# CaptainEven/DenseBox

Hardware: AMD Instinct MI355X
Metric: training patches/sec (240x240) (higher is better)
Workload: dtype f16; 1 GPU; full training step (fwd + fused dense loss w/ hard-negative mining + bwd + grad all-reduce + SGD) of DenseBoxLMLOC on 240x240 patches; net=DenseBoxLMLOC, batch_per_gpu=64, global_batch=64, patch=240x240, parallelism=dp1, half_neg=11, grad_finite=True

## Files before the change

densebox_amd/_lib.py:

```python
import ctypes as C
import os

_HERE = os.path.dirname(os.path.abspath(__file__))
LIB_PATH = os.environ.get('DBX_LIB') or os.path.join(_HERE, 'csrc', 'libdensebox_hip.so')

F16, BF16, F32 = 0, 1, 2
DTYPE_ID = {'f16': F16, 'bf16': BF16, 'f32': F32}
ESIZE = {F16: 2, BF16: 2, F32: 4}

EPI_BIAS, EPI_RELU, EPI_GATE, EPI_DROPMASK, EPI_ACCUM, EPI_F32_NCHW, EPI_DROPHASH = 1, 2, 4, 8, 16, 32, 64
CONV_WFRAG = 128
K_IGEMM, K_DMA, K_BAND, K_C64, K_C8, K_WS, K_P8 = 1, 2, 3, 4, 5, 6, 7


class View(C.Structure):
    _fields_ = [('ptr', C.c_void_p), ('n', C.c_int32), ('h', C.c_int32), ('w', C.c_int32),
                ('pad', C.c_int32), ('ld', C.c_int32), ('c_off', C.c_int32), ('c', C.c_int32)]


class ConvDesc(C.Structure):
    _fields_ = [('dtype', C.c_int32), ('kh', C.c_int32), ('kw', C.c_int32), ('cpad', C.c_int32),
                ('cin_pad', C.c_int32), ('cout_pad', C.c_int32), ('epilogue', C.c_int32), ('drop_seed', C.c_uint32)]


# ... 178 lines not shown
    'dbx_dp_allreduce_sum_f32': (C.c_int, [_VP, _VP, _I64, _VP]),
    'dbx_dp_destroy': (C.c_int, [_VP]),
    'dbx_conv_dgrad_wgrad1_scratch_bytes': (_I64, []),
    'dbx_conv_dgrad_wgrad1_fusable': (C.c_int, [_PC, _PV, _PV, _PV]),
    'dbx_conv_dgrad_wgrad1': (C.c_int, [_PC, _PV, _VP, _PV, _PV, _I32, _VP, _VP, _VP, _I32, _VP]),
    'dbx_conv_pool_fusable': (C.c_int, [_PC, _PV, _PV]),
    'dbx_conv_forward_pool': (C.c_int, [_PC, _PV, _VP, _VP, _PV, _PV, _I32, _VP]),
    'dbx_conv_forward_pool_idx': (C.c_int, [_PC, _PV, _VP, _VP, _PV, _PV, _I32, _VP, _VP]),
    'dbx_pack_weight': (C.c_int, [_I32, _I32, _VP, _I32, _I32, _I32, _I32, _VP, _I32, _I32, _I32, _I32, _VP]),
    'dbx_fold_heads': (C.c_int, [_VP, _VP, _VP, _VP, _I32, _VP, _VP, _VP]),
    'dbx_fold_refine': (C.c_int, [_VP, _VP, _VP, _VP, _VP, _VP, _I32, _I32, _VP, _VP, _VP, _VP]),
    'dbx_refine_eval': (C.c_int, [_VP, _VP, _I32, _I32, _I32, _VP, _VP, _VP, _VP]),
    'dbx_refine_backward_scratch_bytes': (C.c_int64, [_I32, _I32, _I32]),
    'dbx_refine_backward': (C.c_int, [_VP, _VP, _VP, _I32, _I32, _I32, _VP, _VP, _VP, _VP, _VP, _VP, _I32, _VP, _VP, _VP, _VP, _VP, _VP, _VP, _VP, _VP, _VP, _VP, _VP, _VP, _VP]),
    'dbx_upsample_bilinear_nchw_f32': (C.c_int, [_VP, _I32, _I32, _I32, _VP, _I32, _I32, _VP]),
    'dbx_pack_multi': (C.c_int, [_I32, _VP, _I32, _I64, _VP]),
    'dbx_sgd_pack_step': (C.c_int, [_I32, _VP, _I32, _I64, _VP, _F, _F, _F, _I32, _VP]),
    'dbx_head2_dgrad': (C.c_int, [_I32, _PV, C.POINTER(C.c_void_p), C.POINTER(C.c_int32), _I32, _PV, _VP, _I32, _I32, C.c_uint32, _VP]),
    'dbx_head2_wgrad_scratch_bytes': (_I64, [_I32, _I32]),
    'dbx_head2_wgrad': (C.c_int, [_I32, _PV, _PV, C.POINTER(C.c_int32), _I32, C.POINTER(C.c_void_p), C.POINTER(C.c_void_p), _VP, _VP]),
    'dbx_head2_backward': (C.c_int, [_I32, _PV, _PV, C.POINTER(C.c_void_p), C.POINTER(C.c_int32), _I32, _PV, _VP, _I32, _I32, C.c_uint32,
                                     C.POINTER(C.c_void_p), C.POINTER(C.c_void_p), _VP, _VP]),
    'dbx_head2_backward_up': (C.c_int, [_I32, _PV, _PV, C.POINTER(C.c_void_p), C.POINTER(C.c_int32), _I32, _PV, _VP, _I32, _I32, C.c_uint32,
                                        C.POINTER(C.c_void_p), C.POINTER(C.c_void_p), _VP, _PV, _VP]),
    'dbx_perspective_matrix': (C.c_int, [_VP, _VP, _VP]),
    'dbx_warp_perspective_u8': (C.c_int, [_VP, _I32, _I32, _I32, _VP, _VP, _I32, _I32, _VP]),
    'dbx_warp_batch_workspace_bytes': (_I64, [_I32]),
    'dbx_warp_perspective_batch_u8': (C.c_int, [C.POINTER(WarpJob), _I32, _I32, _VP, _VP, _VP]),
    'dbx_plate_crops_batch': (C.c_int, [_VP, _I32, _I32, _VP, _I64, _I64, _VP, _I32, _I32, _I32, _VP, _VP, _VP, _VP]),
    'dbx_match_gt_batch': (C.c_int, [_VP, _I32, _I64, _VP, _VP, _I32, _I32, _VP, _I32, _VP, _VP, _I32, _D, _VP, _VP, _VP, _VP, _VP, _VP]),
# ... 131 lines not shown
```

densebox_amd/csrc/aux_ops.hip:

```cpp
#include "common.hpp"
#include <mutex>

static thread_local char g_err[512] = "";
void dbx_set_error(const char* fmt, ...) {
    va_list ap;
    va_start(ap, fmt);
    vsnprintf(g_err, sizeof(g_err), fmt, ap);
    va_end(ap);
}
extern "C" const char* dbx_last_error(void) { return g_err; }
extern "C" int dbx_version(void) { return DBX_ABI_VERSION; }
extern "C" int dbx_device_arch(int device) {
    hipDeviceProp_t p;
    if (hipGetDeviceProperties(&p, device) != hipSuccess) { dbx_set_error("hipGetDeviceProperties failed"); return DBX_ERR_HIP; }
    int arch = 0;
    const char* s = p.gcnArchName;
    if (s[0] == 'g' && s[1] == 'f' && s[2] == 'x') arch = (int)strtol(s + 3, nullptr, 16) == 0x950 ? 950 : (int)strtol(s + 3, nullptr, 10);
    return arch;
}

template <typename T> struct Vec { static constexpr int N = 16 / sizeof(T); };

template <typename T> __device__ __forceinline__ void load_vec(const T* p, float (&v)[16 / sizeof(T)]) {
    const u32x4 raw = *(const u32x4*)p;
// ... 1809 lines not shown
            const float bot = lx0 * p[y1 * wi + x0] + lx1 * p[y1 * wi + x1];
            y[i] = ly0 * top + ly1 * bot;
        }
    }
}
extern "C" int dbx_upsample_bilinear_nchw_f32(const float* x, int32_t planes, int32_t hi, int32_t wi, float* y, int32_t ho, int32_t wo,
                                              void* stream) {
    DBX_REQUIRE(x && y && planes >= 1 && hi >= 1 && wi >= 1 && ho >= 1 && wo >= 1, "upsample_nchw: bad arguments");
    const int64_t total = (int64_t)planes * ho * wo;
    hipLaunchKernelGGL(upsample_nchw_f32_kernel, dim3(grid_for(total)), dim3(256), 0, (hipStream_t)stream, x, planes, hi, wi, y, ho, wo,
                       ac_scale(hi, ho), ac_scale(wi, wo));
    DBX_LAUNCH_CHECK();
    return DBX_OK;
}

template <typename T>
__global__ void u8hwc_to_framed_kernel(const unsigned char* __restrict__ x, FrameGeo y, float m0, float m1, float m2, float s0,
                                       float s1, float s2) {
    constexpr int V = Vec<T>::N;
    const int cg = y.c / V;
    const int64_t total = (int64_t)y.n * y.h * y.w;
    for (int64_t i = blockIdx.x * (int64_t)blockDim.x + threadIdx.x; i < total; i += (int64_t)gridDim.x * blockDim.x) {
        const int px = (int)(i % y.w);
        const int py = (int)((i / y.w) % y.h);
        const int n = (int)(i / ((int64_t)y.w * y.h));
        const unsigned char* p = x + i * 3;
        float v[3];
        v[0] = ((float)p[0] / 255.0f - m0) / s0;
        v[1] = ((float)p[1] / 255.0f - m1) / s1;
        v[2] = ((float)p[2] / 255.0f - m2) / s2;
// ... 23 lines not shown
```

densebox_amd/csrc/refine_ops.hip:

```cpp
#include "common.hpp"

namespace {
constexpr int RCI = 5, RTAPS = 49, RG1 = RCI * RTAPS + 1;

__device__ __forceinline__ void rf_coef(int d, float scale, int in, int& i0, int& i1, float& l0, float& l1) {
#pragma clang fp contract(off)
    const float src = scale * (float)d;
    i0 = (int)src;
    if (i0 > in - 1) i0 = in - 1;
    i1 = i0 + (i0 < in - 1 ? 1 : 0);
    l1 = src - (float)i0;
    l0 = 1.f - l1;
}
inline float rf_scale(int in, int out) { return out > 1 ? (float)(in - 1) / (float)(out - 1) : 0.f; }

__global__ void refine_up_t_kernel(const float* __restrict__ d, int n, int ho, int wo, float* __restrict__ g, int hs, int ws, float sy, float sx) {
    const int64_t total = (int64_t)n * hs * ws;
    for (int64_t i = blockIdx.x * (int64_t)blockDim.x + threadIdx.x; i < total; i += (int64_t)gridDim.x * blockDim.x) {
        const int px = (int)(i % ws), py = (int)((i / ws) % hs);
        const int64_t im = i / ((int64_t)ws * hs);
        int ylo = sy > 0.f ? (int)((float)(py - 1) / sy) - 1 : 0, yhi = sy > 0.f ? (int)((float)(py + 1) / sy) + 2 : ho - 1;
        int xlo = sx > 0.f ? (int)((float)(px - 1) / sx) - 1 : 0, xhi = sx > 0.f ? (int)((float)(px + 1) / sx) + 2 : wo - 1;
        ylo = ylo < 0 ? 0 : ylo; xlo = xlo < 0 ? 0 : xlo; yhi = yhi > ho - 1 ? ho - 1 : yhi; xhi = xhi > wo - 1 ? wo - 1 : xhi;
        const float* dp = d + im * ho * wo;
        float acc = 0.f;
        for (int y = ylo; y <= yhi; ++y) {
            int y0, y1; float ly0, ly1;
            rf_coef(y, sy, hs, y0, y1, ly0, ly1);
            const float wy = (y0 == py ? ly0 : 0.f) + (y1 == py ? ly1 : 0.f);
            if (wy == 0.f) continue;
            for (int x = xlo; x <= xhi; ++x) {
                int x0, x1; float lx0, lx1;
                rf_coef(x, sx, ws, x0, x1, lx0, lx1);
                const float wx = (x0 == px ? lx0 : 0.f) + (x1 == px ? lx1 : 0.f);
                if (wx != 0.f) acc = fmaf(wy * wx, dp[y * wo + x], acc);
            }
        }
        g[i] = acc;
    }
}

constexpr int RSPLIT = 4;
__global__ __launch_bounds__(256) void refine_g1_kernel(const float* __restrict__ lm, const float* __restrict__ sc, int h, int w,
                                                        const float* __restrict__ g, float* __restrict__ partial) {
    extern __shared__ float sm[];
    const int ph = h / 2, pw = w / 2, oh = ph - 6, ow = pw - 6;
    const int n = blockIdx.x / RSPLIT, part = blockIdx.x % RSPLIT, tid = threadIdx.x;
    const int rows = (oh + RSPLIT - 1) / RSPLIT, y0 = part * rows < oh ? part * rows : oh, y1 = y0 + rows < oh ? y0 + rows : oh;
    const int xr = y1 > y0 ? y1 - y0 + 6 : 0;
    float* x5 = sm;
    float* gs = sm + RCI * (rows + 6) * pw;
    for (int e = tid; e < RCI * xr * pw; e += 256) {
        const int c = e / (xr * pw), r = e % (xr * pw), py = y0 + r / pw, px = r % pw;
// ... 4 lines not shown
    __syncthreads();
    if (tid < RG1) {
        float acc = 0.f;
        if (tid < RCI * RTAPS) {
            const int c = tid / RTAPS, u = (tid % RTAPS) / 7, v = tid % 7;
            const float* xc = x5 + (c * xr + u) * pw + v;
            for (int y = 0; y < y1 - y0; ++y)
                for (int x = 0; x < ow; ++x) acc = fmaf(gs[y * ow + x], xc[y * pw + x], acc);
        } else {
            for (int e = 0; e < (y1 - y0) * ow; ++e) acc += gs[e];
        }
        partial[(size_t)blockIdx.x * RG1 + tid] = acc;
    }
}

struct RefineW { const float *w1, *b1, *w2, *b2, *w3, *b3, *V; float *dw1, *db1, *dw2, *db2, *dw3, *db3; };
__global__ __launch_bounds__(256) void refine_wgrad_kernel(const float* __restrict__ partial, int nimg, int cm, RefineW a) {
    __shared__ float G1[RG1], G2[64 * 25], V[64 * 25], w1s[64 * RCI * 9], red[256];
    const int tid = threadIdx.x;
    for (int e = tid; e < cm * RCI * 9; e += 256) w1s[e] = a.w1[e];
    if (tid < RG1) {
        float acc = 0.f;
#pragma unroll 16
        for (int n = 0; n < nimg; ++n) acc += partial[(size_t)n * RG1 + tid];
        G1[tid] = acc;
    }
    const int blk = blockIdx.x;
    if (blk == cm)
        for (int e = tid; e < cm * 25; e += 256) V[e] = a.V[e];
    __syncthreads();
    const float Sg = G1[RG1 - 1];
    for (int e = tid; e < cm * 25; e += 256) {
        const int m = e / 25, aa = (e % 25) / 5, bb = e % 5;
        float acc = a.b1[m] * Sg;
        for (int c = 0; c < RCI; ++c)
            for (int i = 0; i < 3; ++i)
                for (int j = 0; j < 3; ++j) acc = fmaf(w1s[(m * RCI + c) * 9 + i * 3 + j], G1[(c * 7 + aa + i) * 7 + bb + j], acc);
        G2[e] = acc;
    }
    __syncthreads();
    if (blk < cm) {
        const int n = blk;
// ... 14 lines not shown
    } else {
        for (int e = tid; e < cm * RCI * 9; e += 256) {
            const int m = e / (RCI * 9), c = (e / 9) % RCI, i = (e % 9) / 3, j = e % 3;
            float acc = 0.f;
            for (int aa = 0; aa < 5; ++aa)
                for (int bb = 0; bb < 5; ++bb) acc = fmaf(V[m * 25 + aa * 5 + bb], G1[(c * 7 + aa + i) * 7 + bb + j], acc);
            a.dw1[e] = acc;
        }
        for (int m = tid; m < cm; m += 256) {
            float sv = 0.f;
            for (int ab = 0; ab < 25; ++ab) sv += V[m * 25 + ab];
            a.db1[m] = sv * Sg;
        }
        if (tid == 0) a.db3[0] = Sg;
    }
}

__global__ void refine_dgrad_kernel(const float* __restrict__ lm, const float* __restrict__ sc, int n, int h, int w, const float* __restrict__ g,
                                    const float* __restrict__ wf, const float* __restrict__ g_lm, const float* __restrict__ g_sc,
                                    float* __restrict__ out_lm, float* __restrict__ out_sc) {
    __shared__ float wsm[RCI * RTAPS];
    for (int e = threadIdx.x; e < RCI * RTAPS; e += blockDim.x) wsm[e] = wf[e];
    __syncthreads();
    const int ph = h / 2, pw = w / 2, oh = ph - 6, ow = pw - 6, wh = (h + 1) / 2, ww = (w + 1) / 2;
    const int64_t total = (int64_t)n * RCI * wh * ww;
    for (int64_t i = blockIdx.x * (int64_t)blockDim.x + threadIdx.x; i < total; i += (int64_t)gridDim.x * blockDim.x) {
        const int wx = (int)(i % ww), wy = (int)((i / ww) % wh), c = (int)((i / ((int64_t)ww * wh)) % RCI);
        const int im = (int)(i / ((int64_t)ww * wh * RCI));
        const size_t plane = c < 4 ? ((size_t)im * 4 + c) * h * w : (size_t)im * h * w;
        const float* xin = (c < 4 ? lm : sc) + plane;
// ... 14 lines not shown
            const float* p = xin + (size_t)(2 * wy) * w + 2 * wx;
            float m = p[0]; arg = 0;
            if (p[1] > m) { m = p[1]; arg = 1; }
            if (p[w] > m) { m = p[w]; arg = 2; }
            if (p[w + 1] > m) { m = p[w + 1]; arg = 3; }
        }
#pragma unroll
        for (int k = 0; k < 4; ++k) {
            const int y = 2 * wy + (k >> 1), x = 2 * wx + (k & 1);
            if (y >= h || x >= w) continue;
            const float in = gin ? gin[(size_t)y * w + x] : 0.f;
            dst[(size_t)y * w + x] = in + (k == arg ? dv : 0.f);
        }
    }
}
}

extern "C" int64_t dbx_refine_backward_scratch_bytes(int32_t n, int32_t h, int32_t w) {
    const int64_t oh = h / 2 - 6, ow = w / 2 - 6;
    return ((int64_t)n * oh * ow + (int64_t)n * RSPLIT * RG1 + 64) * 4;
}

extern "C" int dbx_refine_backward(const float* d_refine, const float* landmark, const float* score, int32_t n, int32_t h, int32_t w,
                                   const float* w1, const float* b1, const float* w2, const float* b2, const float* w3, const float* b3,
                                   int32_t cm, const float* w_fold, const float* v_fold, const float* g_landmark, const float* g_score, float* out_landmark,
                                   float* out_score, float* dw1, float* db1, float* dw2, float* db2, float* dw3, float* db3, void* scratch,
                                   void* stream) {
    DBX_REQUIRE(d_refine && landmark && score && w1 && b1 && w2 && b2 && w3 && b3 && w_fold && v_fold && out_landmark && out_score && dw1 && db1 && dw2 &&
                    db2 && dw3 && db3 && scratch, "refine_backward: null argument");
    DBX_REQUIRE(n >= 1 && h / 2 >= 7 && w / 2 >= 7 && cm >= 1 && cm <= 64, "refine_backward: H/2, W/2 >= 7, mid channels <= 64");
// ... 11 lines not shown
    if (attr_once.pending(&attr_dev)) {
        DBX_HIP(hipFuncSetAttribute((const void*)refine_g1_kernel, hipFuncAttributeMaxDynamicSharedMemorySize, 150 * 1024));
        attr_once.mark(attr_dev);
    }
    hipLaunchKernelGGL(refine_g1_kernel, dim3(n * RSPLIT), dim3(256), lds, s, landmark, score, h, w, g, partial);
    DBX_LAUNCH_CHECK();
    RefineW a = {w1, b1, w2, b2, w3, b3, v_fold, dw1, db1, dw2, db2, dw3, db3};
    hipLaunchKernelGGL(refine_wgrad_kernel, dim3(cm + 1), dim3(256), 0, s, partial, n * RSPLIT, cm, a);
    DBX_LAUNCH_CHECK();
    const int64_t tot_d = (int64_t)n * RCI * ((h + 1) / 2) * ((w + 1) / 2);
    hipLaunchKernelGGL(refine_dgrad_kernel, dim3((unsigned)((tot_d + 255) / 256)), dim3(256), 0, s, landmark, score, n, h, w, g, w_fold, g_landmark, g_score,
                       out_landmark, out_score);
    DBX_LAUNCH_CHECK();
    return DBX_OK;
}
```

densebox_amd/engine.py:

```python
import collections
import contextlib
import ctypes as C
import os
import weakref

import torch

from . import _lib
from ._lib import View, ConvDesc, check, ptr, stream_ptr

_BACKBONE = [('conv1_1_1', 3, 64), ('conv1_2_1', 64, 64), ('conv2_1_1', 64, 128), ('conv2_2_1', 128, 128),
             ('conv3_1_1', 128, 256), ('conv3_2_1', 256, 256), ('conv3_4_1', 256, 256),
             ('conv4_1_1', 256, 512), ('conv4_2_1', 512, 512), ('conv4_3_1', 512, 512), ('conv4_4_1', 512, 512)]

_HEADS = {
    'DenseBox': [('det', 1), ('loc', 4)],
    'DenseBoxLM': [('det', 1), ('loc', 4), ('landmark', 4)],
    'DenseBoxLMLOC': [('det', 1), ('loc', 4), ('landmark', 4), ('lmloc', 8)],
}


_FWD_IO = {'conv1_1_1': ('x0', 'a11'), 'conv1_2_1': ('a11', 'a12'), 'conv2_1_1': ('p1', 'a21'), 'conv2_2_1': ('a21', 'a22'),
           'conv3_1_1': ('p2', 'a31'), 'conv3_2_1': ('a31', 'a32'), 'conv3_4_1': ('a32', 'c34'), 'conv4_1_1': ('p3', 'a41'),
           'conv4_2_1': ('a41', 'a42'), 'conv4_3_1': ('a42', 'a43'), 'conv4_4_1': ('a43', 'a44')}
# ... 2 lines not shown
           'conv3_1_1': ('d_a31', 'd_p2'), 'conv2_2_1': ('d_a22', 'd_a21'), 'conv2_1_1': ('d_a21', 'd_p1'),
           'conv1_2_1': ('d_a12', 'd_a11')}
_CH = {s: (ci, co) for s, ci, co in [('conv1_1_1', 3, 64), ('conv1_2_1', 64, 64), ('conv2_1_1', 64, 128), ('conv2_2_1', 128, 128),
                                     ('conv3_1_1', 128, 256), ('conv3_2_1', 256, 256), ('conv3_4_1', 256, 256),
                                     ('conv4_1_1', 256, 512), ('conv4_2_1', 512, 512), ('conv4_3_1', 512, 512),
                                     ('conv4_4_1', 512, 512)]}


Image = collections.namedtuple('Image', 'key srcs dt mode kh kw rows_pad cin_pad place')
PackJob = collections.namedtuple('PackJob', 'src dst co ci taps mode ktot cin_pad row_off k_off rows_lim')
_TNAME = ('f16', 'bf16', 'f32')


def _align(x, a=256):
    return (x + a - 1) // a * a


class Buf:

    def __init__(self, name, n, h, w, c, pad, dtype_id):
        self.name, self.n, self.h, self.w, self.c, self.pad = name, n, h, w, c, pad
        self.dtype_id = dtype_id
        self.es = _lib.ESIZE[dtype_id]
        self.hp, self.wp = h + 2 * pad, w + 2 * pad
        self.bytes = n * self.hp * self.wp * c * self.es
        self.guard = _align(max(4 * (self.wp + 2), 576 + 4 * self.wp) * c * self.es)
        self.base = None

    def view(self, c_off=0, c=None):
        return View(C.c_void_p(self.base), self.n, self.h, self.w, self.pad, self.c, c_off,
# ... 664 lines not shown
            o = 0
            for stem, k in heads:
                if big is not None:
                    outs[stem] = big[:, o:o + k].contiguous()
                o += k
        P.refine_fwd = None
        rf_convs = ('conv6_1_det', 'f') in P.manifest
        if kind != 'DenseBox' and not rf_convs:
            wf7, bf7, vf7 = self._w_refine_folded()
            lmk, det = outs['landmark'], outs['det']
            if not lmk.is_contiguous():
                lmk = lmk.contiguous()
            if not det.is_contiguous():
                det = det.contiguous()
            small = torch.empty((n, 1, h4 // 2 - 6, w4 // 2 - 6), dtype=torch.float32, device=dev)
            check(L.dbx_refine_eval(ptr(lmk), ptr(det), n, h4, w4, ptr(wf7), ptr(bf7), ptr(small), s))
            o = torch.empty((n, 1, h4, w4), dtype=torch.float32, device=dev)
            check(L.dbx_upsample_bilinear_nchw_f32(ptr(small), n, h4 // 2 - 6, w4 // 2 - 6, ptr(o), h4, w4, s))
            outs['refine'] = o
            if train:
                P.refine_fwd = (lmk, det, wf7, vf7)
        elif kind != 'DenseBox':
            rdt = P.rdt
            w61, w62, w63 = (self._fetch(P, (st, 'f'))[0] for st in ('conv6_1_det', 'conv6_2_det', 'conv6_3_det'))
            rin = B['rf_in'].view()
            check(L.dbx_nchw_to_framed_ch(rdt, ptr(outs['landmark']), 4, C.byref(rin), 0, s))
            check(L.dbx_nchw_to_framed_ch(rdt, ptr(outs['det']), 1, C.byref(rin), 4, s))
            check(L.dbx_maxpool2x2(rdt, C.byref(rin), C.byref(B['rf_p'].view()), s))
            self._conv(rdt, B['rf_p'].view(), B['rf_1'].view(), w61,
                       self._fetch(P, ('conv6_1_det', 'bias'))[0], 3, 3, 0, P.crf, 64, _lib.EPI_BIAS, alg_ci=5)
            self._conv(rdt, B['rf_1'].view(), B['rf_2'].view(), w62,
                       self._fetch(P, ('conv6_2_det', 'bias'))[0], 5, 5, 0, 64, 64, _lib.EPI_BIAS)
            check(L.dbx_upsample_bilinear(rdt, C.byref(B['rf_2'].view()), C.byref(B['rf_u'].view()), s))
# ... 131 lines not shown
        def dgrad(stem, src, dst, kh, kw, cpad, rows_pad, cin_pad, gate=None, epi=0, dropmask=None):
            wp, wfrag = self._fetch(P, (stem, 'b'))
            e = epi | (_lib.EPI_GATE if gate is not None else 0) | wfrag
            self._conv(dt, src, dst, wp, None, kh, kw, cpad, cin_pad, rows_pad, e, gate=gate, dropmask=dropmask,
                       dm_ld=512 * nh)

        override = {}
        if kind != 'DenseBox' and P.refine_fwd is not None:
            lmk, det, wf7, vf7 = P.refine_fwd
            pn = ['conv6_1_det.weight', 'conv6_1_det.bias', 'conv6_2_det.weight', 'conv6_2_det.bias', 'conv6_3_det.weight', 'conv6_3_det.bias']
            ps = [self._param(nm).detach() for nm in pn]
            gs = [new_grad(nm) for nm in pn]

            def f32c(t):
                return None if t is None else t.to(torch.float32).contiguous()
            g_lm, g_det = f32c(grad_outs.get('landmark')), f32c(grad_outs.get('det'))
            o_lm = torch.empty((n, 4, h4, w4), dtype=torch.float32, device=dev)
            o_det = torch.empty((n, 1, h4, w4), dtype=torch.float32, device=dev)
            need = L.dbx_refine_backward_scratch_bytes(n, h4, w4)
            if getattr(self, '_rf_scratch', None) is None or self._rf_scratch.numel() < need:
                self._rf_scratch = torch.empty(int(need), dtype=torch.uint8, device=dev)
            d_rf = gout('refine', 1)
            check(L.dbx_refine_backward(ptr(d_rf), ptr(lmk), ptr(det), n, h4, w4, *[ptr(p) for p in ps], ps[0].shape[0], ptr(wf7), ptr(vf7),
                                        ptr(g_lm), ptr(g_det), ptr(o_lm), ptr(o_det), *[ptr(g_) for g_ in gs], ptr(self._rf_scratch), s))
            if sink is not None:
                sink.ready(pn)
            override = {'landmark': o_lm, 'det': o_det}
        elif kind != 'DenseBox' and ('conv6_1_det', 'b') not in M:
            raise RuntimeError('densebox_amd: backward of the refine branch without its forward state (no training-mode forward on this plan)')
        elif kind != 'DenseBox':
            d_rfo = B['d_rfo'].view()
            check(L.dbx_nchw_to_framed(dt, ptr(gout('refine', 1)), 1, C.byref(d_rfo), s))
            conv_bwd('conv6_3_det', d_rfo, B['rf_u'].view(), 1, 1, 0, 1, 64)
            dgrad('conv6_3_det', d_rfo, B['d_rf_u'].view(), 1, 1, 0, 64, P.crf)
            check(L.dbx_upsample_bilinear_bwd(dt, C.byref(B['d_rf_u'].view()), C.byref(B['d_rf_2'].view()), None, s))
            conv_bwd('conv6_2_det', B['d_rf_2'].view(), B['rf_1'].view(), 5, 5, 0, 64, 64)
            dgrad('conv6_2_det', B['d_rf_2'].view(), B['d_rf_1'].view(), 5, 5, 4, 64, 64)
            conv_bwd('conv6_1_det', B['d_rf_1'].view(), B['rf_p'].view(), 3, 3, 0, 64, 5)
            dgrad('conv6_1_det', B['d_rf_1'].view(), B['d_rf_p'].view(), 3, 3, 2, 64, 64)
            check(L.dbx_maxpool2x2_bwd(dt, C.byref(B['rf_in'].view()), C.byref(B['d_rf_p'].view()),
                                       C.byref(B['d_rf_in'].view()), 0, 0, s))

        slot = {}
        srcs = []
        for i, (stem, k) in enumerate(heads):
            slot[stem] = B['d_out'].view(P.crf * i, P.crf)
            src = override.get(stem)
            srcs.append(src if src is not None else gout(stem, k))
        if override or kind == 'DenseBox':
            check(L.dbx_nchw_to_framed_slots(dt, (C.c_void_p * nh)(*[t.data_ptr() for t in srcs]), (C.c_int32 * nh)(*[k for _, k in heads]), nh, P.crf,
                                             C.byref(B['d_out'].view()), s))
        else:
            for (stem, k), t in zip(heads, srcs):
                check(L.dbx_nchw_to_framed(dt, ptr(t), k, C.byref(slot[stem]), s))
        if kind != 'DenseBox' and not override:
            check(L.dbx_framed_add_ch(dt, C.byref(B['d_rf_in'].view()), 0, 4, C.byref(slot['landmark']), 0, s))
            check(L.dbx_framed_add_ch(dt, C.byref(B['d_rf_in'].view()), 4, 1, C.byref(slot['det']), 0, s))

        hv = B['hid'].view()
        need = L.dbx_head2_wgrad_scratch_bytes(nh, hv.n * hv.h)
        if getattr(self, '_h2_scratch', None) is None or self._h2_scratch.numel() < need:
            self._h2_scratch = torch.empty(int(need), dtype=torch.uint8, device=dev)
        dw2 = [new_grad('conv5_2_%s.weight' % st) for st, _ in heads]
        db2 = [new_grad('conv5_2_%s.bias' % st) for st, _ in heads]
# ... 163 lines not shown
```

densebox_amd/loss.py:

```python
import ctypes as C

import numpy as np
import torch

from . import _lib, labels as LB
from ._lib import LossDesc, LossIO, check, ptr, stream_ptr

_KIND_ID = {'DenseBox': 0, 'DenseBoxLM': 1, 'DenseBoxLMLOC': 2}


class _LossFn(torch.autograd.Function):
    @staticmethod
    def forward(ctx, loss, n_out, *outs_and_grads):
        outs, grads = outs_and_grads[:n_out], outs_and_grads[n_out:]
        ctx.grads = grads
        return loss.clone()

    @staticmethod
    def backward(ctx, g):
        return (None, None) + tuple(d * g for d in ctx.grads) + (None,) * len(ctx.grads)


def densebox_loss(kind, outputs, bbox, vertices=None, labels=None, rand_neg_indices=None, lm_rand_neg_indices=None,
                  lambda_loc=3.0, lambda_det=1.0, lambda_lm=0.5, batch_global=None, positive_num_global=None,
                  return_debug=False, rng=None):
    kid = _KIND_ID[kind]
    if kind == 'DenseBox':
        score, loc = outputs
        lm = rf = lmloc = None
    elif kind == 'DenseBoxLM':
        score, loc, lm, rf = outputs
# ... 58 lines not shown
```

include/densebox_hip.h:

```cpp
#ifndef DENSEBOX_HIP_H
#define DENSEBOX_HIP_H

#include <stdint.h>

#ifdef __cplusplus
extern "C" {
#endif

enum dbx_status {
    DBX_OK = 0,
    DBX_ERR_ARG = -1,
    DBX_ERR_HIP = -2,
    DBX_ERR_DTYPE = -3
};

enum dbx_dtype { DBX_F16 = 0, DBX_BF16 = 1, DBX_F32 = 2 };

const char* dbx_last_error(void);
#define DBX_ABI_VERSION 13
int dbx_version(void);
int dbx_device_arch(int device);

typedef struct dbx_view {
    void*   ptr;
// ... 101 lines not shown

int dbx_fold_heads(const float* w2, const float* b2, const float* w1, const float* b1, int32_t k, float* w_out,
                   float* b_out, void* stream);
int dbx_fold_refine(const float* w1, const float* b1, const float* w2, const float* b2, const float* w3, const float* b3,
                    int32_t ci, int32_t cm, float* w_out, float* b_out, float* v_out, void* stream);
int dbx_refine_eval(const float* landmark_nchw, const float* score_nchw, int32_t n, int32_t h, int32_t w, const float* w_fold,
                    const float* b_fold, float* out_small, void* stream);
int dbx_upsample_bilinear_nchw_f32(const float* x, int32_t planes, int32_t hi, int32_t wi, float* y, int32_t ho, int32_t wo,
                                   void* stream);
int64_t dbx_refine_backward_scratch_bytes(int32_t n, int32_t h, int32_t w);
int dbx_refine_backward(const float* d_refine, const float* landmark, const float* score, int32_t n, int32_t h, int32_t w,
                        const float* w1, const float* b1, const float* w2, const float* b2, const float* w3, const float* b3,
                        int32_t cm, const float* w_fold, const float* v_fold, const float* g_landmark, const float* g_score, float* out_landmark,
                        float* out_score, float* dw1, float* db1, float* dw2, float* db2, float* dw3, float* db3, void* scratch,
                        void* stream);

int64_t dbx_conv_wgrad_scratch_bytes(int32_t dtype, const dbx_view* dz, const dbx_view* x, int32_t kh, int32_t kw);
int dbx_conv_wgrad(int32_t dtype, const dbx_view* dz, const dbx_view* x, int32_t kh, int32_t kw, int32_t cpad,
                   int32_t co, int32_t ci, float* dw_oihw, float* db, void* scratch, int32_t accumulate, void* stream);
int dbx_conv_wgrad_slice(int32_t dtype, const dbx_view* dz, const dbx_view* x, int32_t kh, int32_t kw, int32_t cpad,
                         int32_t co, int32_t ci, float* dw_oihw, int32_t dw_ci_total, int32_t dw_ci_off, float* db, void* scratch,
                         int32_t accumulate, void* stream);
int dbx_conv_wgrad_plan(int32_t dtype, const dbx_view* dz, const dbx_view* x, int32_t kh, int32_t kw, char* name, int32_t name_len,
                        int32_t* splits);

int64_t dbx_conv_dgrad_wgrad1_scratch_bytes(void);
int dbx_conv_dgrad_wgrad1_fusable(const dbx_conv_desc* d, const dbx_view* dz, const dbx_view* gate, const dbx_view* x0);
int dbx_conv_dgrad_wgrad1(const dbx_conv_desc* d, const dbx_view* dz, const void* w_packed, const dbx_view* gate, const dbx_view* x0,
                          int32_t ci, float* dw_oihw, float* db, void* scratch, int32_t accumulate, void* stream);

// ... 388 lines not shown
```

Before: 7543 patches/s.

## Fuse refine branch forward and backward chains into banded LDS kernels

Forward fuses refine eval (pool + 7x7 conv) with the bilinear upsample into one banded kernel that keeps the small map in LDS. Backward fuses the upsample-transpose with the first-layer wgrad partials, then merges the weight-grad blocks with a dgrad kernel. That kernel writes the landmark/score gradients, including the max-pool scatter, straight into the framed d_out slots. This drops the intermediate f32 NCHW tensors and the separate nchw_to_framed_slots pass. The loss clone is also replaced by a view. Risks are recomputed pooling in each band, heavier LDS use and more complex indexing.

```diff
diff --git a/densebox_amd/_lib.py b/densebox_amd/_lib.py
--- a/densebox_amd/_lib.py
+++ b/densebox_amd/_lib.py
@@ -216,6 +216,10 @@
     'dbx_refine_backward_scratch_bytes': (C.c_int64, [_I32, _I32, _I32]),
     'dbx_refine_backward': (C.c_int, [_VP, _VP, _VP, _I32, _I32, _I32, _VP, _VP, _VP, _VP, _VP, _VP, _I32, _VP, _VP, _VP, _VP, _VP, _VP, _VP, _VP, _VP, _VP, _VP, _VP, _VP, _VP]),
     'dbx_upsample_bilinear_nchw_f32': (C.c_int, [_VP, _I32, _I32, _I32, _VP, _I32, _I32, _VP]),
+    'dbx_refine_forward': (C.c_int, [_VP, _VP, _I32, _I32, _I32, _VP, _VP, _VP, _VP, _VP]),
+    'dbx_refine_backward_slots': (C.c_int, [_I32, _VP, _VP, _VP, _I32, _I32, _I32, _VP, _VP, _VP, _VP, _VP, _VP, _I32, _VP, _VP,
+                                            C.POINTER(C.c_void_p), C.POINTER(C.c_int32), _I32, _I32, _I32, _I32, _PV,
+                                            _VP, _VP, _VP, _VP, _VP, _VP, _VP, _VP]),
     'dbx_pack_multi': (C.c_int, [_I32, _VP, _I32, _I64, _VP]),
     'dbx_sgd_pack_step': (C.c_int, [_I32, _VP, _I32, _I64, _VP, _F, _F, _F, _I32, _VP]),
     'dbx_head2_dgrad': (C.c_int, [_I32, _PV, C.POINTER(C.c_void_p), C.POINTER(C.c_int32), _I32, _PV, _VP, _I32, _I32, C.c_uint32, _VP]),
diff --git a/densebox_amd/csrc/aux_ops.hip b/densebox_amd/csrc/aux_ops.hip
--- a/densebox_amd/csrc/aux_ops.hip
+++ b/densebox_amd/csrc/aux_ops.hip
@@ -1847,6 +1847,71 @@
     return DBX_OK;
 }
 
+constexpr int RF_ROWS = 16, RF_SMAX = RF_ROWS / 2 + 2, RF_WPAD = 248;
+static inline size_t refine_forward_lds(int w) { return ((size_t)RF_WPAD + (size_t)5 * (RF_SMAX + 6) * (w / 2) + (size_t)RF_SMAX * (w / 2 - 6)) * 4; }
+__global__ __launch_bounds__(256) void refine_forward_kernel(const float* __restrict__ lm, const float* __restrict__ sc, int h, int w, int bands,
+                                                             const float* __restrict__ wf, const float* __restrict__ bf, float* __restrict__ out,
+                                                             float sy, float sx) {
+    constexpr int CI = 5;
+    extern __shared__ float rsm[];
+    const int pw = w / 2, oh = h / 2 - 6, ow = pw - 6;
+    const int n = blockIdx.x / bands, r0 = (blockIdx.x % bands) * RF_ROWS, r1 = r0 + RF_ROWS < h ? r0 + RF_ROWS : h, tid = threadIdx.x;
+    int slo, shi, t;
+    float l0, l1;
+    bilin_coef(r0, sy, oh, slo, t, l0, l1);
+    bilin_coef(r1 - 1, sy, oh, t, shi, l0, l1);
+    const int sr = shi - slo + 1, xr = sr + 6;
+    float* wsm = rsm;
+    float* x5 = rsm + RF_WPAD;
+    float* ss = x5 + CI * (RF_SMAX + 6) * pw;
+    for (int e = tid; e < CI * 49; e += 256) wsm[e] = wf[e];
+    for (int e = tid; e < CI * xr * pw; e += 256) {
+        const int c = e / (xr * pw), r = e % (xr * pw), py = slo + r / pw, px = r % pw;
+        const float* p = (c < 4 ? lm + ((size_t)n * 4 + c) * h * w : sc + (size_t)n * h * w) + (size_t)(2 * py) * w + 2 * px;
+        x5[e] = fmaxf(fmaxf(p[0], p[1]), fmaxf(p[w], p[w + 1]));
+    }
+    __syncthreads();
+    for (int e = tid; e < sr * ow; e += 256) {
+        const int ty = e / ow, tx = e % ow;
+        float acc = bf[0];
+        for (int c = 0; c < CI; ++c)
+#pragma unroll
+            for (int u = 0; u < 7; ++u)
+#pragma unroll
+                for (int v = 0; v < 7; ++v) acc = fmaf(wsm[(c * 7 + u) * 7 + v], x5[(c * xr + ty + u) * pw + tx + v], acc);
+        ss[e] = acc;
+    }
+    __syncthreads();
+    for (int e = tid; e < (r1 - r0) * w; e += 256) {
+        const int py = r0 + e / w, px = e % w;
+        int y0, y1, x0, x1;
+        float ly0, ly1, lx0, lx1;
+        bilin_coef(py, sy, oh, y0, y1, ly0, ly1);
+        bilin_coef(px, sx, ow, x0, x1, lx0, lx1);
+        {
+#pragma clang fp contract(off)
+            const float top = lx0 * ss[(y0 - slo) * ow + x0] + lx1 * ss[(y0 - slo) * ow + x1];
+            const float bot = lx0 * ss[(y1 - slo) * ow + x0] + lx1 * ss[(y1 - slo) * ow + x1];
+            out[((size_t)n * h + py) * w + px] = ly0 * top + ly1 * bot;
+        }
+    }
+}
+extern "C" int dbx_refine_forward(const float* landmark_nchw, const float* score_nchw, int32_t n, int32_t h, int32_t w, const float* w_fold,
+                                  const float* b_fold, float* small, float* out, void* stream) {
+    DBX_REQUIRE(landmark_nchw && score_nchw && w_fold && b_fold && small && out && n >= 1 && h / 2 >= 7 && w / 2 >= 7,
+                "refine_forward: bad arguments (H/2, W/2 >= 7)");
+    const int oh = h / 2 - 6, ow = w / 2 - 6, bands = (h + RF_ROWS - 1) / RF_ROWS;
+    const size_t lds = refine_forward_lds(w);
+    if (lds > 64 * 1024 || (int64_t)n * bands >= (1ll << 31)) {
+        const int rc = dbx_refine_eval(landmark_nchw, score_nchw, n, h, w, w_fold, b_fold, small, stream);
+        return rc != DBX_OK ? rc : dbx_upsample_bilinear_nchw_f32(small, n, oh, ow, out, h, w, stream);
+    }
+    hipLaunchKernelGGL(refine_forward_kernel, dim3((unsigned)(n * bands)), dim3(256), lds, (hipStream_t)stream, landmark_nchw, score_nchw, h, w, bands,
+                       w_fold, b_fold, out, ac_scale(oh, h), ac_scale(ow, w));
+    DBX_LAUNCH_CHECK();
+    return DBX_OK;
+}
+
 template <typename T>
 __global__ void u8hwc_to_framed_kernel(const unsigned char* __restrict__ x, FrameGeo y, float m0, float m1, float m2, float s0,
                                        float s1, float s2) {
diff --git a/densebox_amd/csrc/refine_ops.hip b/densebox_amd/csrc/refine_ops.hip
--- a/densebox_amd/csrc/refine_ops.hip
+++ b/densebox_amd/csrc/refine_ops.hip
@@ -14,29 +14,35 @@
 }
 inline float rf_scale(int in, int out) { return out > 1 ? (float)(in - 1) / (float)(out - 1) : 0.f; }
 
+__device__ __forceinline__ void up_t_window(int p, float s, int out, int& lo, int& hi) {
+    lo = s > 0.f ? (int)((float)(p - 1) / s) - 1 : 0; hi = s > 0.f ? (int)((float)(p + 1) / s) + 2 : out - 1;
+    lo = lo < 0 ? 0 : lo; hi = hi > out - 1 ? out - 1 : hi;
+}
+__device__ __forceinline__ float up_t_elem(const float* dp, int row0, int py, int px, int ho, int wo, int hs, int ws, float sy, float sx) {
+    int ylo, yhi, xlo, xhi;
+    up_t_window(py, sy, ho, ylo, yhi);
+    up_t_window(px, sx, wo, xlo, xhi);
+    float acc = 0.f;
+    for (int y = ylo; y <= yhi; ++y) {
+        int y0, y1; float ly0, ly1;
+        rf_coef(y, sy, hs, y0, y1, ly0, ly1);
+        const float wy = (y0 == py ? ly0 : 0.f) + (y1 == py ? ly1 : 0.f);
+        if (wy == 0.f) continue;
+        for (int x = xlo; x <= xhi; ++x) {
+            int x0, x1; float lx0, lx1;
+            rf_coef(x, sx, ws, x0, x1, lx0, lx1);
+            const float wx = (x0 == px ? lx0 : 0.f) + (x1 == px ? lx1 : 0.f);
+            if (wx != 0.f) acc = fmaf(wy * wx, dp[(y - row0) * wo + x], acc);
+        }
+    }
+    return acc;
+}
 __global__ void refine_up_t_kernel(const float* __restrict__ d, int n, int ho, int wo, float* __restrict__ g, int hs, int ws, float sy, float sx) {
     const int64_t total = (int64_t)n * hs * ws;
     for (int64_t i = blockIdx.x * (int64_t)blockDim.x + threadIdx.x; i < total; i += (int64_t)gridDim.x * blockDim.x) {
         const int px = (int)(i % ws), py = (int)((i / ws) % hs);
         const int64_t im = i / ((int64_t)ws * hs);
-        int ylo = sy > 0.f ? (int)((float)(py - 1) / sy) - 1 : 0, yhi = sy > 0.f ? (int)((float)(py + 1) / sy) + 2 : ho - 1;
-        int xlo = sx > 0.f ? (int)((float)(px - 1) / sx) - 1 : 0, xhi = sx > 0.f ? (int)((float)(px + 1) / sx) + 2 : wo - 1;
-        ylo = ylo < 0 ? 0 : ylo; xlo = xlo < 0 ? 0 : xlo; yhi = yhi > ho - 1 ? ho - 1 : yhi; xhi = xhi > wo - 1 ? wo - 1 : xhi;
-        const float* dp = d + im * ho * wo;
-        float acc = 0.f;
-        for (int y = ylo; y <= yhi; ++y) {
-            int y0, y1; float ly0, ly1;
-            rf_coef(y, sy, hs, y0, y1, ly0, ly1);
-            const float wy = (y0 == py ? ly0 : 0.f) + (y1 == py ? ly1 : 0.f);
-            if (wy == 0.f) continue;
-            for (int x = xlo; x <= xhi; ++x) {
-                int x0, x1; float lx0, lx1;
-                rf_coef(x, sx, ws, x0, x1, lx0, lx1);
-                const float wx = (x0 == px ? lx0 : 0.f) + (x1 == px ? lx1 : 0.f);
-                if (wx != 0.f) acc = fmaf(wy * wx, dp[y * wo + x], acc);
-            }
-        }
-        g[i] = acc;
+        g[i] = up_t_elem(d + im * ho * wo, 0, py, px, ho, wo, hs, ws, sy, sx);
     }
 }
 
@@ -71,8 +77,52 @@
     }
 }
 
+__global__ __launch_bounds__(256) void refine_g1_up_kernel(const float* __restrict__ lm, const float* __restrict__ sc, int h, int w,
+                                                           const float* __restrict__ d, float sy, float sx, int dcap, float* __restrict__ g,
+                                                           float* __restrict__ partial) {
+    extern __shared__ float sm[];
+    const int ph = h / 2, pw = w / 2, oh = ph - 6, ow = pw - 6;
+    const int n = blockIdx.x / RSPLIT, part = blockIdx.x % RSPLIT, tid = threadIdx.x;
+    const int rows = (oh + RSPLIT - 1) / RSPLIT, y0 = part * rows < oh ? part * rows : oh, y1 = y0 + rows < oh ? y0 + rows : oh;
+    const int xr = y1 > y0 ? y1 - y0 + 6 : 0;
+    float* x5 = sm;
+    float* gs = sm + RCI * (rows + 6) * pw;
+    float* ds = gs + rows * ow;
+    const float* dn = d + (size_t)n * h * w;
+    int dlo = 0, dhi = -1;
+    if (y1 > y0) { int t; up_t_window(y0, sy, h, dlo, t); up_t_window(y1 - 1, sy, h, t, dhi); }
+    const bool staged = dhi - dlo + 1 <= dcap;
+    if (staged)
+        for (int e = tid; e < (dhi - dlo + 1) * w; e += 256) ds[e] = dn[(size_t)dlo * w + e];
+    for (int e = tid; e < RCI * xr * pw; e += 256) {
+        const int c = e / (xr * pw), r = e % (xr * pw), py = y0 + r / pw, px = r % pw;
+        const float* p = (c < 4 ? lm + ((size_t)n * 4 + c) * h * w : sc + (size_t)n * h * w) + (size_t)(2 * py) * w + 2 * px;
+        x5[e] = fmaxf(fmaxf(p[0], p[1]), fmaxf(p[w], p[w + 1]));
+    }
+    __syncthreads();
+    for (int e = tid; e < (y1 - y0) * ow; e += 256) {
+        const int py = y0 + e / ow, px = e % ow;
+        const float acc = staged ? up_t_elem(ds, dlo, py, px, h, w, oh, ow, sy, sx) : up_t_elem(dn, 0, py, px, h, w, oh, ow, sy, sx);
+        gs[e] = acc;
+        g[((size_t)n * oh + y0) * ow + e] = acc;
+    }
+    __syncthreads();
+    if (tid < RG1) {
+        float acc = 0.f;
+        if (tid < RCI * RTAPS) {
+            const int c = tid / RTAPS, u = (tid % RTAPS) / 7, v = tid % 7;
+            const float* xc = x5 + (c * xr + u) * pw + v;
+            for (int y = 0; y < y1 - y0; ++y)
+                for (int x = 0; x < ow; ++x) acc = fmaf(gs[y * ow + x], xc[y * pw + x], acc);
+        } else {
+            for (int e = 0; e < (y1 - y0) * ow; ++e) acc += gs[e];
+        }
+        partial[(size_t)blockIdx.x * RG1 + tid] = acc;
+    }
+}
+
 struct RefineW { const float *w1, *b1, *w2, *b2, *w3, *b3, *V; float *dw1, *db1, *dw2, *db2, *dw3, *db3; };
-__global__ __launch_bounds__(256) void refine_wgrad_kernel(const float* __restrict__ partial, int nimg, int cm, RefineW a) {
+__device__ __forceinline__ void refine_wgrad_body(const float* __restrict__ partial, int nimg, int cm, const RefineW& a, const int blk) {
     __shared__ float G1[RG1], G2[64 * 25], V[64 * 25], w1s[64 * RCI * 9], red[256];
     const int tid = threadIdx.x;
     for (int e = tid; e < cm * RCI * 9; e += 256) w1s[e] = a.w1[e];
@@ -82,7 +132,6 @@
         for (int n = 0; n < nimg; ++n) acc += partial[(size_t)n * RG1 + tid];
         G1[tid] = acc;
     }
-    const int blk = blockIdx.x;
     if (blk == cm)
         for (int e = tid; e < cm * 25; e += 256) V[e] = a.V[e];
     __syncthreads();
@@ -127,6 +176,9 @@
         }
         if (tid == 0) a.db3[0] = Sg;
     }
+}
+__global__ __launch_bounds__(256) void refine_wgrad_kernel(const float* __restrict__ partial, int nimg, int cm, RefineW a) {
+    refine_wgrad_body(partial, nimg, cm, a, blockIdx.x);
 }
 
 __global__ void refine_dgrad_kernel(const float* __restrict__ lm, const float* __restrict__ sc, int n, int h, int w, const float* __restrict__ g,
@@ -171,6 +223,87 @@
         }
     }
 }
+
+struct RefineSlots { const float* x[4]; int k[4]; int nslots, slot, lm_slot, det_slot; };
+template <typename T> __device__ __forceinline__ void rf_store_vec(T* p, const float (&v)[16 / sizeof(T)]) {
+    u32x4 raw;
+    T* e = (T*)&raw;
+#pragma unroll
+    for (int i = 0; i < 16 / (int)sizeof(T); ++i) e[i] = from_f32<T>(v[i]);
+    *(u32x4*)p = raw;
+}
+__device__ __forceinline__ void rf_dgrad_taps(const float* wsm, const float* gp, int oh, int ow, int wy, int wx, int cb, int nc, float (&dv)[4]) {
+    for (int u = 0; u < 7; ++u) {
+        const int y = wy - u;
+        if (y < 0 || y >= oh) continue;
+        for (int v = 0; v < 7; ++v) {
+            const int x = wx - v;
+            if (x < 0 || x >= ow) continue;
+            const float gv = gp[y * ow + x];
+#pragma unroll
+            for (int c = 0; c < 4; ++c)
+                if (c < nc) dv[c] = fmaf(wsm[((cb + c) * 7 + u) * 7 + v], gv, dv[c]);
+        }
+    }
+}
+template <typename T>
+__global__ __launch_bounds__(256) void refine_bwd_slots_kernel(const float* __restrict__ partial, int nimg, int cm, RefineW a, const float* __restrict__ lm,
+                                                               const float* __restrict__ sc, int h, int w, const float* __restrict__ g,
+                                                               const float* __restrict__ wf, RefineSlots ss, FrameGeo yv, int bpi, int g_lds) {
+    extern __shared__ float gsm[];
+    if ((int)blockIdx.x <= cm) { refine_wgrad_body(partial, nimg, cm, a, (int)blockIdx.x); return; }
+    __shared__ float wsm[RCI * RTAPS];
+    constexpr int V = 16 / (int)sizeof(T);
+    const int tid = threadIdx.x, b = (int)blockIdx.x - (cm + 1), im = b / bpi, chunk = b % bpi;
+    const int ph = h / 2, pw = w / 2, oh = ph - 6, ow = pw - 6, wh = (h + 1) / 2, ww = (w + 1) / 2;
+    const float* gim = g + (size_t)im * oh * ow;
+    for (int e = tid; e < RCI * RTAPS; e += 256) wsm[e] = wf[e];
+    if (g_lds)
+        for (int e = tid; e < oh * ow; e += 256) gsm[e] = gim[e];
+    __syncthreads();
+    const int gps = ss.slot / V, cg = ss.nslots * gps;
+    const int i = chunk * 256 + tid;
+    if (i >= wh * ww * cg) return;
+    const int wx = i % ww, gi = (i / ww) % cg, wy = i / (ww * cg);
+    const int si = gi / gps, c0 = (gi % gps) * V;
+    const float* xs = si == 0 ? ss.x[0] : si == 1 ? ss.x[1] : si == 2 ? ss.x[2] : ss.x[3];
+    const int kk = si == 0 ? ss.k[0] : si == 1 ? ss.k[1] : si == 2 ? ss.k[2] : ss.k[3];
+    const bool rf = si == ss.lm_slot || si == ss.det_slot;
+    float dv[4] = {0.f, 0.f, 0.f, 0.f};
+    int arg[4] = {-1, -1, -1, -1};
+    if (rf && c0 == 0 && wy < ph && wx < pw) {
+        const int cb = si == ss.lm_slot ? 0 : 4, nc = si == ss.lm_slot ? 4 : 1;
+        if (g_lds) rf_dgrad_taps(wsm, gsm, oh, ow, wy, wx, cb, nc, dv);
+        else rf_dgrad_taps(wsm, gim, oh, ow, wy, wx, cb, nc, dv);
+#pragma unroll
+        for (int c = 0; c < 4; ++c) {
+            if (c >= nc) continue;
+            const float* p = (cb + c < 4 ? lm + ((size_t)im * 4 + c) * h * w : sc + (size_t)im * h * w) + (size_t)(2 * wy) * w + 2 * wx;
+            float m = p[0]; int ar = 0;
+            if (p[1] > m) { m = p[1]; ar = 1; }
+            if (p[w] > m) { m = p[w]; ar = 2; }
+            if (p[w + 1] > m) { m = p[w + 1]; ar = 3; }
+            arg[c] = ar;
+        }
+    }
+#pragma unroll
+    for (int k = 0; k < 4; ++k) {
+        const int y = 2 * wy + (k >> 1), x = 2 * wx + (k & 1);
+        if (y >= h || x >= w) continue;
+        float v[V];
+#pragma unroll
+        for (int j = 0; j < V; ++j) {
+            const int c = c0 + j;
+            float val = 0.f;
+            if (c < kk) {
+                const float in = xs ? xs[(((size_t)im * kk + c) * h + y) * w + x] : 0.f;
+                val = rf ? in + ((j < 4 && k == arg[j < 4 ? j : 0]) ? dv[j < 4 ? j : 0] : 0.f) : in;
+            }
+            v[j] = val;
+        }
+        rf_store_vec<T>((T*)yv.base + geo_pix(yv, im, y, x) + si * ss.slot + c0, v);
+    }
+}
 }
 
 extern "C" int64_t dbx_refine_backward_scratch_bytes(int32_t n, int32_t h, int32_t w) {
@@ -212,3 +345,72 @@
     DBX_LAUNCH_CHECK();
     return DBX_OK;
 }
+
+namespace {
+struct RefineBwdArgs {
+    const float *d_refine, *landmark, *score;
+    int n, h, w, cm;
+    RefineW a;
+    const float* w_fold;
+    RefineSlots ss;
+    void* scratch;
+};
+template <typename T> int refine_backward_slots_t(const RefineBwdArgs& r, const dbx_view* y, hipStream_t s) {
+    constexpr int V = 16 / (int)sizeof(T);
+    DBX_REQUIRE(((size_t)y->ptr % 16) == 0 && (y->ld * sizeof(T)) % 16 == 0 && (y->c_off * sizeof(T)) % 16 == 0 && r.ss.slot % V == 0,
+                "refine_backward_slots: view must be 16-byte aligned/strided, slots a multiple of the vector width");
+    const int n = r.n, h = r.h, w = r.w, ph = h / 2, pw = w / 2, oh = ph - 6, ow = pw - 6;
+    const int rows = (oh + RSPLIT - 1) / RSPLIT;
+    const size_t lds0 = ((size_t)RCI * (rows + 6) * pw + (size_t)rows * ow) * 4;
+    DBX_REQUIRE(lds0 <= 150 * 1024, "refine_backward_slots: map too large for the per-image LDS tile (%d x %d)", h, w);
+    const float sy = rf_scale(oh, h), sx = rf_scale(ow, w);
+    int64_t dcap = sy > 0.f ? (int64_t)((float)(rows + 1) / sy) + 6 : h;
+    if (dcap > h) dcap = h;
+    if (lds0 + (size_t)dcap * w * 4 > 150 * 1024) dcap = 0;
+    const size_t lds = lds0 + (size_t)dcap * w * 4;
+    float* g = (float*)r.scratch;
+    float* partial = g + (size_t)n * oh * ow;
+    static DbxDevOnce attr_once; int attr_dev = 0;
+    if (attr_once.pending(&attr_dev)) {
+        DBX_HIP(hipFuncSetAttribute((const void*)refine_g1_up_kernel, hipFuncAttributeMaxDynamicSharedMemorySize, 150 * 1024));
+        attr_once.mark(attr_dev);
+    }
+    hipLaunchKernelGGL(refine_g1_up_kernel, dim3(n * RSPLIT), dim3(256), lds, s, r.landmark, r.score, h, w, r.d_refine, sy, sx, (int)dcap, g, partial);
+    DBX_LAUNCH_CHECK();
+    FrameGeo geo = make_geo<T>(y);
+    const int cg = r.ss.nslots * (r.ss.slot / V);
+    const int64_t per = (int64_t)((h + 1) / 2) * ((w + 1) / 2) * cg;
+    const int bpi = (int)((per + 255) / 256);
+    DBX_REQUIRE((int64_t)n * bpi + r.cm + 1 < (1ll << 31), "refine_backward_slots: too many workgroups");
+    const int g_lds = (size_t)oh * ow * 4 <= 32 * 1024;
+    hipLaunchKernelGGL(refine_bwd_slots_kernel<T>, dim3((unsigned)(r.cm + 1 + n * bpi)), dim3(256), g_lds ? (size_t)oh * ow * 4 : 0, s, partial, n * RSPLIT,
+                       r.cm, r.a, r.landmark, r.score, h, w, g, r.w_fold, r.ss, geo, bpi, g_lds);
+    DBX_LAUNCH_CHECK();
+    return DBX_OK;
+}
+}
+
+extern "C" int dbx_refine_backward_slots(int32_t dtype, const float* d_refine, const float* landmark, const float* score, int32_t n, int32_t h, int32_t w,
+                                         const float* w1, const float* b1, const float* w2, const float* b2, const float* w3, const float* b3,
+                                         int32_t cm, const float* w_fold, const float* v_fold, const float* const* g_heads, const int32_t* k,
+                                         int32_t nslots, int32_t slot, int32_t lm_slot, int32_t det_slot, const dbx_view* d_out, float* dw1, float* db1,
+                                         float* dw2, float* db2, float* dw3, float* db3, void* scratch, void* stream) {
+    DBX_REQUIRE(d_refine && landmark && score && w1 && b1 && w2 && b2 && w3 && b3 && w_fold && v_fold && g_heads && k && d_out && d_out->ptr && dw1 && db1 &&
+                    dw2 && db2 && dw3 && db3 && scratch, "refine_backward_slots: null argument");
+    DBX_REQUIRE(n >= 1 && h / 2 >= 7 && w / 2 >= 7 && cm >= 1 && cm <= 64, "refine_backward_slots: H/2, W/2 >= 7, mid channels <= 64");
+    DBX_REQUIRE(nslots >= 2 && nslots <= 4 && slot >= 4 && d_out->c == nslots * slot && d_out->c_off + d_out->c <= d_out->ld,
+                "refine_backward_slots: 2..4 slots, view of nslots * slot channels");
+    DBX_REQUIRE(d_out->n == n && d_out->h == h && d_out->w == w && d_out->pad >= 0, "refine_backward_slots: d_out must have the maps' geometry");
+    DBX_REQUIRE(lm_slot >= 0 && lm_slot < nslots && det_slot >= 0 && det_slot < nslots && lm_slot != det_slot && k[lm_slot] == 4 && k[det_slot] == 1,
+                "refine_backward_slots: landmark (k = 4) and score (k = 1) slots");
+    RefineBwdArgs r;
+    r.d_refine = d_refine; r.landmark = landmark; r.score = score; r.n = n; r.h = h; r.w = w; r.cm = cm;
+    r.a = {w1, b1, w2, b2, w3, b3, v_fold, dw1, db1, dw2, db2, dw3, db3};
+    r.w_fold = w_fold; r.scratch = scratch;
+    r.ss.nslots = nslots; r.ss.slot = slot; r.ss.lm_slot = lm_slot; r.ss.det_slot = det_slot;
+    for (int i = 0; i < 4; ++i) {
+        r.ss.x[i] = i < nslots ? g_heads[i] : nullptr; r.ss.k[i] = i < nslots ? k[i] : 0;
+        if (i < nslots) DBX_REQUIRE(k[i] >= 0 && k[i] <= slot, "refine_backward_slots: k must fit its slot");
+    }
+    DBX_DISPATCH_DTYPE(dtype, refine_backward_slots_t, r, d_out, (hipStream_t)stream);
+}
diff --git a/densebox_amd/engine.py b/densebox_amd/engine.py
--- a/densebox_amd/engine.py
+++ b/densebox_amd/engine.py
@@ -40,6 +40,10 @@
 
 def _align(x, a=256):
     return (x + a - 1) // a * a
+
+
+def _step_chain():
+    return os.environ.get('DBX_STEP_CHAIN', '1') != '0'
 
 
 class Buf:
@@ -734,9 +738,12 @@
             if not det.is_contiguous():
                 det = det.contiguous()
             small = torch.empty((n, 1, h4 // 2 - 6, w4 // 2 - 6), dtype=torch.float32, device=dev)
-            check(L.dbx_refine_eval(ptr(lmk), ptr(det), n, h4, w4, ptr(wf7), ptr(bf7), ptr(small), s))
             o = torch.empty((n, 1, h4, w4), dtype=torch.float32, device=dev)
-            check(L.dbx_upsample_bilinear_nchw_f32(ptr(small), n, h4 // 2 - 6, w4 // 2 - 6, ptr(o), h4, w4, s))
+            if _step_chain():
+                check(L.dbx_refine_forward(ptr(lmk), ptr(det), n, h4, w4, ptr(wf7), ptr(bf7), ptr(small), ptr(o), s))
+            else:
+                check(L.dbx_refine_eval(ptr(lmk), ptr(det), n, h4, w4, ptr(wf7), ptr(bf7), ptr(small), s))
+                check(L.dbx_upsample_bilinear_nchw_f32(ptr(small), n, h4 // 2 - 6, w4 // 2 - 6, ptr(o), h4, w4, s))
             outs['refine'] = o
             if train:
                 P.refine_fwd = (lmk, det, wf7, vf7)
@@ -898,18 +905,27 @@
 
             def f32c(t):
                 return None if t is None else t.to(torch.float32).contiguous()
-            g_lm, g_det = f32c(grad_outs.get('landmark')), f32c(grad_outs.get('det'))
-            o_lm = torch.empty((n, 4, h4, w4), dtype=torch.float32, device=dev)
-            o_det = torch.empty((n, 1, h4, w4), dtype=torch.float32, device=dev)
             need = L.dbx_refine_backward_scratch_bytes(n, h4, w4)
             if getattr(self, '_rf_scratch', None) is None or self._rf_scratch.numel() < need:
                 self._rf_scratch = torch.empty(int(need), dtype=torch.uint8, device=dev)
             d_rf = gout('refine', 1)
-            check(L.dbx_refine_backward(ptr(d_rf), ptr(lmk), ptr(det), n, h4, w4, *[ptr(p) for p in ps], ps[0].shape[0], ptr(wf7), ptr(vf7),
-                                        ptr(g_lm), ptr(g_det), ptr(o_lm), ptr(o_det), *[ptr(g_) for g_ in gs], ptr(self._rf_scratch), s))
+            if _step_chain():
+                ins = [f32c(grad_outs.get(stem)) for stem, _ in heads]
+                stems = [stem for stem, _ in heads]
+                check(L.dbx_refine_backward_slots(dt, ptr(d_rf), ptr(lmk), ptr(det), n, h4, w4, *[ptr(p) for p in ps], ps[0].shape[0], ptr(wf7), ptr(vf7),
+                                                  (C.c_void_p * nh)(*[t.data_ptr() if t is not None else None for t in ins]),
+                                                  (C.c_int32 * nh)(*[k for _, k in heads]), nh, P.crf, stems.index('landmark'), stems.index('det'),
+                                                  C.byref(B['d_out'].view()), *[ptr(g_) for g_ in gs], ptr(self._rf_scratch), s))
+                override = {'landmark': None, 'det': None}
+            else:
+                g_lm, g_det = f32c(grad_outs.get('landmark')), f32c(grad_outs.get('det'))
+                o_lm = torch.empty((n, 4, h4, w4), dtype=torch.float32, device=dev)
+                o_det = torch.empty((n, 1, h4, w4), dtype=torch.float32, device=dev)
+                check(L.dbx_refine_backward(ptr(d_rf), ptr(lmk), ptr(det), n, h4, w4, *[ptr(p) for p in ps], ps[0].shape[0], ptr(wf7), ptr(vf7),
+                                            ptr(g_lm), ptr(g_det), ptr(o_lm), ptr(o_det), *[ptr(g_) for g_ in gs], ptr(self._rf_scratch), s))
+                override = {'landmark': o_lm, 'det': o_det}
             if sink is not None:
                 sink.ready(pn)
-            override = {'landmark': o_lm, 'det': o_det}
         elif kind != 'DenseBox' and ('conv6_1_det', 'b') not in M:
             raise RuntimeError('densebox_amd: backward of the refine branch without its forward state (no training-mode forward on this plan)')
         elif kind != 'DenseBox':
@@ -927,11 +943,15 @@
 
         slot = {}
         srcs = []
+        in_slots = bool(override) and override['landmark'] is None
         for i, (stem, k) in enumerate(heads):
             slot[stem] = B['d_out'].view(P.crf * i, P.crf)
             src = override.get(stem)
-            srcs.append(src if src is not None else gout(stem, k))
-        if override or kind == 'DenseBox':
+            if not in_slots:
+                srcs.append(src if src is not None else gout(stem, k))
+        if in_slots:
+            pass
+        elif override or kind == 'DenseBox':
             check(L.dbx_nchw_to_framed_slots(dt, (C.c_void_p * nh)(*[t.data_ptr() for t in srcs]), (C.c_int32 * nh)(*[k for _, k in heads]), nh, P.crf,
                                              C.byref(B['d_out'].view()), s))
         else:
diff --git a/densebox_amd/loss.py b/densebox_amd/loss.py
--- a/densebox_amd/loss.py
+++ b/densebox_amd/loss.py
@@ -14,7 +14,7 @@
     def forward(ctx, loss, n_out, *outs_and_grads):
         outs, grads = outs_and_grads[:n_out], outs_and_grads[n_out:]
         ctx.grads = grads
-        return loss.clone()
+        return loss.view_as(loss)
 
     @staticmethod
     def backward(ctx, g):
diff --git a/include/densebox_hip.h b/include/densebox_hip.h
--- a/include/densebox_hip.h
+++ b/include/densebox_hip.h
@@ -139,6 +139,13 @@
                         int32_t cm, const float* w_fold, const float* v_fold, const float* g_landmark, const float* g_score, float* out_landmark,
                         float* out_score, float* dw1, float* db1, float* dw2, float* db2, float* dw3, float* db3, void* scratch,
                         void* stream);
+int dbx_refine_forward(const float* landmark_nchw, const float* score_nchw, int32_t n, int32_t h, int32_t w, const float* w_fold,
+                       const float* b_fold, float* small, float* out, void* stream);
+int dbx_refine_backward_slots(int32_t dtype, const float* d_refine, const float* landmark, const float* score, int32_t n, int32_t h, int32_t w,
+                              const float* w1, const float* b1, const float* w2, const float* b2, const float* w3, const float* b3,
+                              int32_t cm, const float* w_fold, const float* v_fold, const float* const* g_heads, const int32_t* k,
+                              int32_t nslots, int32_t slot, int32_t lm_slot, int32_t det_slot, const dbx_view* d_out, float* dw1, float* db1,
+                              float* dw2, float* db2, float* dw3, float* db3, void* scratch, void* stream);
 
 int64_t dbx_conv_wgrad_scratch_bytes(int32_t dtype, const dbx_view* dz, const dbx_view* x, int32_t kh, int32_t kw);
 int dbx_conv_wgrad(int32_t dtype, const dbx_view* dz, const dbx_view* x, int32_t kh, int32_t kw, int32_t cpad,
```

Result: no change. 7503 patches/s (-0.5%).
